# GothiProCoder/OCR-System

Hardware: AMD Instinct MI355X
Metric: pages/sec end-to-end det+rec, A4@200DPI (higher is better)
Workload: dtype bf16; 1 GPU; end-to-end det+rec, batch=64 A4@200DPI pages per GPU (BASELINE configs[3]); pages_per_gpu=64, global_batch=64, lines_last_step=3279, pages_gathered_last_step=64, parallelism=pages sharded dp1, 1 all-gather/step, ranks=1, input=pages pre-decoded (uint8 RGB) and resident in HBM when the timed region starts, det_sub_batch=64

## Files before the change

### ocr-system_amd/csrc/capi.hip

```cpp
#include <cstdlib>
#include <cstring>
#include <new>

#include "../../include/lumina_ocr.h"
#include "dbpost.h"
#include "deskew.h"
#include "engine.h"
#include "ops.h"
#include "resize.h"
#include "jpeg.h"
#include "jpegdec.h"
#include "stem_conv.h"

#define API_TRY try {
#define API_CATCH(h)                                                             \
    }                                                                            \
    catch (const std::exception& e) { return locr_fail(h, "exception", e.what()); } \
    catch (...) { return locr_fail(h, "exception", "unknown"); }

namespace {
struct DeviceGuard {
    int prev = -1;
    hipError_t err;
    explicit DeviceGuard(int dev) {
// ... 13 lines not shown

static int hip_rc(lumina_ocr* h, const char* what, hipError_t e) { return e == hipSuccess ? 0 : locr_fail(h, what, hipGetErrorString(e)); }

template <class F> static int drain_launches(lumina_ocr* h, const char* what, F&& f) {
    if (hipDeviceSynchronize() != hipSuccess) return locr_fail(h, what, "sync failed");
    for (const LaunchRecord& r : h->launches) {
        float t = 0.f;
        if (hipEventElapsedTime(&t, r.e0.get(), r.e1.get()) != hipSuccess) t = 0.f;
        f(r, t);
    }
    h->launches.clear();
    return 0;
}

extern "C" {

const char* lumina_ocr_version(void) { return "lumina-ocr-mi355x 0.1 (gfx950)"; }

int lumina_ocr_create(int device, lumina_ocr_t** out) {
    if (!out) return 1;
    *out = nullptr;
    lumina_ocr* eng = new (std::nothrow) lumina_ocr();
    if (!eng) return 1;
    eng->device = device;
    int ndev = 0;
    if (hipGetDeviceCount(&ndev) != hipSuccess || device < 0 || device >= ndev) {
        eng->err = "no HIP device " + std::to_string(device) + " (device count " + std::to_string(ndev) + ")";
        *out = eng;
        return 2;
    }
    if (hipSetDevice(device) != hipSuccess) { eng->err = "hipSetDevice failed"; *out = eng; return 2; }
    if (const char* e = getenv("LUMINA_RING_ORIENT")) eng->ring_orient = atoi(e) < 0 ? -1 : (atoi(e) != 0);
    if (getenv("LUMINA_CONV_NO_RING")) eng->conv_ring = false;
    if (getenv("LUMINA_BLOCKED")) eng->blocked_layout = atoi(getenv("LUMINA_BLOCKED")) != 0;
    *out = eng;
    return 0;
}

void lumina_ocr_destroy(lumina_ocr_t* h) {
    if (!h) return;
    (void)hipSetDevice(h->device);
    delete h;
}

const char* lumina_ocr_last_error(const lumina_ocr_t* h) { return h ? h->err.c_str() : "null handle"; }

int lumina_ocr_set_option(lumina_ocr_t* h, const char* key, int value) {
    if (!h || !key) return 1;
    if (!strcmp(key, "det_sub_batch")) h->det_sub_batch = value > 0 ? value : 1;
    else if (!strcmp(key, "rec_sub_batch")) h->rec_sub_batch = value > 0 ? value : 1;
    else if (!strcmp(key, "keep_taps")) h->keep_taps = value < 0 || value > 2 ? 0 : value;
    else if (!strcmp(key, "time_convs")) h->time_convs = value != 0;
    else if (!strcmp(key, "fuse_head")) h->fuse_head = value != 0;
    else if (!strcmp(key, "fuse_mb")) h->fuse_mb = value != 0;
    else if (!strcmp(key, "fuse_pool")) h->fuse_pool = value != 0;
    else if (!strcmp(key, "fuse_stem")) h->fuse_stem = value != 0;
    else if (!strcmp(key, "fpn_multi")) h->fpn_multi = value != 0;
    else if (!strcmp(key, "fpn_compose")) h->fpn_compose = value != 0;
    else if (!strcmp(key, "fuse_short")) h->fuse_short = value != 0;
    else if (!strcmp(key, "conv_ring")) h->conv_ring = value != 0;
    else if (!strcmp(key, "blocked_layout")) h->blocked_layout = value != 0;
    else if (!strcmp(key, "conv_big_min")) h->conv_big_min = value >= 0 ? value : 1024;
    else if (!strcmp(key, "ring_orient")) h->ring_orient = value < 0 ? -1 : (value != 0);
    else if (!strcmp(key, "post_group")) h->post_group = value > 0 ? value : 1;
    else if (!strcmp(key, "tail_group")) h->tail_group = value > 0 ? value : 0;
    else if (!strcmp(key, "svtr_f16")) h->svtr_f16 = value < 0 ? -1 : (value != 0);
    else if (!strcmp(key, "conv2d_variant")) h->conv2d_variant = value < 0 || value > 2 ? 0 : value;
    else return locr_fail(h, "set_option: unknown key", key);
    return 0;
}

int lumina_ocr_load_det_weights(lumina_ocr_t* h, const void* blob, size_t nbytes) {
    if (!h || !blob) return 1;
    BIND(h);
    API_TRY return eng_load_det(h, blob, nbytes); API_CATCH(h)
}
int lumina_ocr_load_rec_weights(lumina_ocr_t* h, const void* blob, size_t nbytes) {
    if (!h || !blob) return 1;
    BIND(h);
    API_TRY return eng_load_rec(h, blob, nbytes); API_CATCH(h)
}
int lumina_ocr_num_classes(const lumina_ocr_t* h) { return h ? h->num_classes : 0; }

int lumina_ocr_normalize(lumina_ocr_t* h, const uint8_t* img_dev, int n, int height, int width, int hp, int wp, const float scale[3],
                         const float shift[3], int layout_nchw, uint16_t* out_dev, void* stream) {
    if (!h || !img_dev || !out_dev || hp < height || wp < width) return locr_fail(h, "normalize", "bad arguments");
    BIND(h);
    return hip_rc(h, "normalize", normalize_launch(img_dev, out_dev, n, height, width, hp, wp, height, width, scale, shift, layout_nchw, (hipStream_t)stream));
}

int lumina_ocr_det_forward(lumina_ocr_t* h, const uint8_t* pages_dev, int batch, int height, int width, int hp, int wp, uint16_t* prob_dev,
                           void* stream) {
    if (!h || !pages_dev || !prob_dev) return locr_fail(h, "det_forward", "null argument");
// ... 327 lines not shown
```

### ocr-system_amd/csrc/conv_mfma.h

```cpp
#pragma once
#include "common.h"

enum ConvOutMode : int {
    OUT_NORMAL = 0,
    OUT_UPSAMPLE = 1,
    OUT_CONVT = 2,
    OUT_CONVT1 = 3,
    OUT_POOL = 4,
};

struct ConvParams {
    const bf16_t* x;
    const bf16_t* wpk;
    const float* bias;
    const bf16_t* res;
    bf16_t* y;
    int N, H, W, Cin;
    int Ho, Wo;
    int Cout;
    int y_cstride, y_coff;
    int res_cstride, res_h, res_w, res_shift;
    int act;
    int out_mode, up_shift, convt_c;
    int tiles_x, tiles_y, n_tiles;
// ... 1 lines not shown
    float fuse_b;
    const bf16_t* gate;
    int gate_hw;
    int dbg_skip;
    int pix_limit;
    const bf16_t* zeros;
    int x_blk, y_blk, res_blk;
    int n_src;
    const bf16_t* xs[4];
    int xs_shift[4];
    int xs_nchunk[4], xs_cstride[4];
    const bf16_t* wpk2;
    const float* bias2;
    bf16_t* y2;
    int y2_cstride;
};

struct ConvKernelCfg {
    int ks, stride, bn, ck, tw, nw;
};

size_t conv_packed_weight_elems(int cout_gemm, int ks, int cin, int bn);
void pack_conv_weights(const bf16_t* ohwi, int cout_gemm, int ks, int cin, int bn, int ck, bf16_t* out, int row_major = 0);

bool conv_pick_cfg(int ks, int stride, int cin, int cout_gemm, ConvKernelCfg* cfg);
hipError_t conv_launch(const ConvKernelCfg& cfg, ConvParams p, hipStream_t stream);
const char* conv_kernel_name(const ConvKernelCfg& cfg);

bool conv_ring_supported(const ConvKernelCfg& cfg, const ConvParams& p);
bool conv_ring_transposed(const ConvParams& p, int orientation);
hipError_t conv_ring_launch(ConvParams p, int orientation, hipStream_t stream);
const char* conv_ring_kernel_name(const ConvParams& p, int orientation);

bool conv_pw_supported(const ConvKernelCfg& cfg, const ConvParams& p);
hipError_t conv_pw_launch(const ConvParams& p, hipStream_t stream);
```

### ocr-system_amd/csrc/engine.h

```cpp
#pragma once
#include <map>
#include <memory>
#include <string>
#include <type_traits>
#include <vector>

#include "common.h"
#include "conv_mfma.h"
#include "mbconv.h"
#include "svtr.h"

struct Tensor4 {
    bf16_t* p = nullptr;
    int n = 0, h = 0, w = 0, c = 0;
    bool blk = false;
    int n_src = 0; const bf16_t* xs[4] = {nullptr, nullptr, nullptr, nullptr}; int xs_shift[4] = {0, 0, 0, 0};
    int xs_c[4] = {0, 0, 0, 0}, xs_cs[4] = {0, 0, 0, 0};
    int src_c(int k) const { return xs_c[k] ? xs_c[k] : c / n_src; }
    int src_cs(int k) const { return xs_cs[k] ? xs_cs[k] : src_c(k); }
    size_t elems() const { return (size_t)n * h * w * c; }
};

struct ConvLayer {
    std::string name;
    int ks = 1, stride = 1, cin = 0, cout = 0;
    int act = ACT_NONE;
    bool convt = false;
    int convt_c = 0;
    ConvKernelCfg cfg{};
    bf16_t* wpk = nullptr;
    ConvKernelCfg cfg_big{}; bf16_t* wpk_big = nullptr;
    bool force_big = false;
    int launch_group = 0;
    bool small_only = false;
    bf16_t* fuse_w = nullptr; float fuse_b = 0.f;
    double alg_flop_per_px = 0;
    float* bias = nullptr;
};

struct DwLayer { int k = 3, c = 0; bf16_t* w = nullptr; float* bias = nullptr; };
struct SeLayer { int c = 0, mid = 0; bf16_t *w1 = nullptr, *w2 = nullptr; float *b1 = nullptr, *b2 = nullptr; };

struct RecBlock {
    int k, cin, exp, cout, se_mid, stride_h, act;
    bool se, res;
    ConvLayer expand, project;
    DwLayer dw;
    bf16_t* we_pk = nullptr; float* be_pk = nullptr;
    SeLayer sel;
};

struct SvtrLinear {
    int K = 0, N = 0, taps = 1, cin = 0, act = ACT_NONE;
    uint16_t* w = nullptr;
    float* bias = nullptr;
    float *gamma = nullptr, *beta = nullptr;
};
struct SvtrBlock { int dim = 0, heads = 0, gh = 0, gw = 0; bool local = false; SvtrLinear qkv, proj, fc1, fc2; };
struct SvtrModel {
    bool loaded = false;
    int dtype = 0;
    int dims[3] = {64, 128, 256}, depths[3] = {3, 6, 3}, heads[3] = {2, 4, 8}, local_blocks = 6, out_ch = 192;
    int num_classes = 0, ctc_ntiles = 0;
    SvtrLinear pe1, pe2, sub[2], last;
// ... 31 lines not shown
struct HostBlobTensor { int dtype; std::vector<int> dims; const uint8_t* data; size_t nbytes; };

struct lumina_ocr {
    int device = 0;
    std::string err;
    bool det_loaded = false;
    std::map<std::string, ConvLayer> det;
    bf16_t* stem_wpk = nullptr; float* stem_bias = nullptr;
    bool rec_loaded = false;
    int num_classes = 0, ctc_ntiles = 0;
    bf16_t* rstem_wpk = nullptr; float* rstem_bias = nullptr;
    std::vector<RecBlock> rblocks;
    ConvLayer rconv2, xproj[2];
    bf16_t* whh[2] = {nullptr, nullptr};
    bf16_t* ctc_wpk = nullptr; float* ctc_bias = nullptr;
    SvtrModel svtr;
    Growable<DeviceMem> ws;
    Arena arena;
    std::vector<DeviceMem> owned;
    bf16_t* zeros = nullptr;
    int det_sub_batch = 16, rec_sub_batch = 4096, post_group = 64;
    int tail_group = 16;
    std::map<std::string, Tensor4> taps;
    int keep_taps = 0;
    bool fuse_head = true;
    bool fuse_pool = true;
    int conv_big_min = 1024;
    bool blocked_layout = true;
    bool conv_ring = true;
    int svtr_f16 = -1;
    int conv2d_variant = 0;
    int ring_orient = -1;
    bool fuse_short = true;
    bool fpn_compose = true;
    bool fpn_multi = true;
    bool fuse_stem = true;
    bool fuse_mb = true;
    bool time_convs = false;
    std::vector<LaunchRecord> launches;
    struct Coeffs { int ksize = 0; int* bounds = nullptr; int* kk = nullptr; std::shared_ptr<std::vector<int>> bounds_host; };
    std::map<std::pair<int, int>, Coeffs> coeff_cache;
    Growable<DeviceMem> aux;
    Growable<DeviceMem> sums;
    int jd_last_passes = 0;
    struct Staging { Growable<PinnedMem> buf; Event uploaded; };
    Staging jd_stage[2];
    int jd_stage_next = 0;
    float* dk_trig = nullptr; short* dk_wtab = nullptr;
};

int locr_fail(lumina_ocr* eng, const char* what, const char* detail);
bool parse_blob(lumina_ocr* eng, const void* blob, size_t n, std::map<std::string, HostBlobTensor>* out);

int eng_load_det(lumina_ocr* eng, const void* blob, size_t n);
int eng_load_rec(lumina_ocr* eng, const void* blob, size_t n);
int eng_det_forward(lumina_ocr* eng, const uint8_t* pages, int B, int H, int W, int Hp, int Wp, bf16_t* prob, hipStream_t st);
int eng_rec_forward(lumina_ocr* eng, const uint8_t* crops, const int* widths, int N, int* idx, float* prob, hipStream_t st);
int eng_load_svtr(lumina_ocr* eng, const void* blob, size_t n);
int eng_svtr_forward(lumina_ocr* eng, const uint8_t* crops, const int* widths, int N, int* idx, float* prob, hipStream_t st);
int eng_ws_reserve(lumina_ocr* eng, size_t bytes);
void* eng_upload(lumina_ocr* eng, const void* host, size_t bytes);
int eng_run_conv(lumina_ocr* eng, const ConvLayer& L, const Tensor4& x, Tensor4* y, const Tensor4* res, int res_shift, int out_mode,
                 int up_shift, int y_cstride, int y_coff, bool flat, hipStream_t st, const bf16_t* gate = nullptr,
                 const ConvLayer* short_l = nullptr, Tensor4* short_y = nullptr);
```

### ocr-system_amd/csrc/engine.hip

```cpp
#include "engine.h"

#include <cstdlib>
#include <cstring>

#include "ops.h"
#include "stem_conv.h"

int locr_fail(lumina_ocr* eng, const char* what, const char* detail) {
    if (eng) eng->err = std::string(what) + ": " + (detail ? detail : "");
    return 1;
}

#include <mutex>
#include <set>
hipError_t locr_dyn_lds(const void* kernel, int bytes) {
    static std::mutex mu;
    static std::set<std::pair<int, const void*>> done;
    int dev = 0;
    hipError_t e = hipGetDevice(&dev);
    if (e != hipSuccess) return e;
    std::lock_guard<std::mutex> lk(mu);
    if (done.count({dev, kernel})) return hipSuccess;
    e = hipFuncSetAttribute(kernel, hipFuncAttributeMaxDynamicSharedMemorySize, bytes);
    if (e == hipSuccess) done.insert({dev, kernel});
// ... 72 lines not shown
        locr_fail(eng, "missing/ill-typed tensor", name.c_str());
        return false;
    }
    *w = &iw->second; *b = &ib->second;
    return true;
}

static bool make_conv(lumina_ocr* eng, const std::map<std::string, HostBlobTensor>& m, const std::string& name, int ks, int stride,
                      int cin_r, int cout_r, int cin_p, int cout_p, int act, ConvLayer* L, int bias_repeat = 1) {
    const HostBlobTensor *w, *b;
    if (!get_wb(eng, m, name, &w, &b)) return false;
    if (w->dims.size() != 4 || w->dims[0] != cout_r || w->dims[1] != ks || w->dims[3] != cin_r ||
        (int)b->dims[0] * bias_repeat != cout_r) {
        locr_fail(eng, "unexpected tensor shape", name.c_str());
        return false;
    }
    L->name = name; L->ks = ks; L->stride = stride; L->cin = cin_p; L->cout = cout_p; L->act = act;
    if (!conv_pick_cfg(ks, stride, cin_p, cout_p, &L->cfg)) { locr_fail(eng, "no conv kernel config", name.c_str()); return false; }
    const int taps = ks * ks;
    std::vector<bf16_t> padded((size_t)cout_p * taps * cin_p, 0);
    const bf16_t* src = reinterpret_cast<const bf16_t*>(w->data);
    for (int co = 0; co < cout_r; ++co)
        for (int t = 0; t < taps; ++t)
            memcpy(&padded[((size_t)co * taps + t) * cin_p], &src[((size_t)co * taps + t) * cin_r], sizeof(bf16_t) * cin_r);
    std::vector<bf16_t> packed(conv_packed_weight_elems(cout_p, ks, cin_p, L->cfg.bn));
    pack_conv_weights(padded.data(), cout_p, ks, cin_p, L->cfg.bn, L->cfg.ck, packed.data());
    L->wpk = static_cast<bf16_t*>(eng_upload(eng, packed.data(), packed.size() * sizeof(bf16_t)));
    static const int dma = getenv("LUMINA_CONV_DMA") != nullptr ? atoi(getenv("LUMINA_CONV_DMA")) : 1;
    if (ks == 3 && stride == 1 && L->cfg.bn == 64 && (cin_p >= 64 || name == "stem.conv3") && L->cfg.nw == 4) {
        L->cfg_big = L->cfg; L->cfg_big.nw = dma ? 6 : 5; L->cfg_big.ck = 16;
        std::vector<bf16_t> packed2(conv_packed_weight_elems(cout_p, ks, cin_p, 64));
        pack_conv_weights(padded.data(), cout_p, ks, cin_p, 64, 16, packed2.data(), dma ? 1 : 0);
        L->wpk_big = static_cast<bf16_t*>(eng_upload(eng, packed2.data(), packed2.size() * sizeof(bf16_t)));
    }
    const int ntiles = (cout_p + L->cfg.bn - 1) / L->cfg.bn;
    std::vector<float> bias((size_t)ntiles * L->cfg.bn, 0.f);
    const float* bs = reinterpret_cast<const float*>(b->data);
    const int bn_r = b->dims[0];
    for (int i = 0; i < cout_r; ++i) bias[i] = bs[i % bn_r];
    L->bias = static_cast<float*>(eng_upload(eng, bias.data(), bias.size() * sizeof(float)));
    if (!L->wpk || !L->bias) { locr_fail(eng, "device upload failed", name.c_str()); return false; }
    return true;
}

static inline float host_bf16_to_f32(bf16_t b) { uint32_t u = (uint32_t)b << 16; float f; memcpy(&f, &u, 4); return f; }
static inline bf16_t host_f32_to_bf16(float f) {
    uint32_t u; memcpy(&u, &f, 4);
    return (bf16_t)((u + 0x7fffu + ((u >> 16) & 1u)) >> 16);
}

static int compose_fpn_p2(lumina_ocr* eng, const std::map<std::string, HostBlobTensor>& m) {
    const HostBlobTensor *wi, *bi, *wp, *bp;
    if (!get_wb(eng, m, "fpn.in2", &wi, &bi) || !get_wb(eng, m, "fpn.p2", &wp, &bp)) return 1;
    const float* b_in2 = reinterpret_cast<const float*>(bi->data);
    for (int i = 0; i < 256; ++i)
        if (b_in2[i] != 0.f) return 0;
    const bf16_t* Wi = reinterpret_cast<const bf16_t*>(wi->data);
    const bf16_t* Wp = reinterpret_cast<const bf16_t*>(wp->data);
    std::vector<bf16_t> w((size_t)64 * 9 * 320);
    std::vector<double> win((size_t)256 * 64);
    for (size_t i = 0; i < win.size(); ++i) win[i] = (double)host_bf16_to_f32(Wi[i]);
    for (int co = 0; co < 64; ++co)
        for (int t = 0; t < 9; ++t) {
            double acc[64] = {0};
            const bf16_t* row = Wp + ((size_t)co * 9 + t) * 256;
            for (int mm = 0; mm < 256; ++mm) {
// ... 59 lines not shown
        ConvLayer& L3 = eng->det["head.convt3"];
        if (!make_conv(eng, m, "head.convt3", 1, 1, 64, 4, 64, 4, ACT_SIGMOID, &L3, 4)) return 1;
        L3.convt = true; L3.convt_c = 1;
        const HostBlobTensor *w3, *b3;
        if (!get_wb(eng, m, "head.convt3", &w3, &b3)) return 1;
        ConvLayer& Lf = eng->det["head.convt2.fused"];
        Lf = L;
        Lf.name = "head.convt2+3";
        {
            const bf16_t* w3s = reinterpret_cast<const bf16_t*>(w3->data);
            std::vector<bf16_t> img(4 * 2 * 32 * 8, 0);
            for (int ks = 0; ks < 4; ++ks)
                for (int hh = 0; hh < 2; ++hh)
                    for (int row = 0; row < 4; ++row)
                        for (int j = 0; j < 8; ++j) img[((ks * 2 + hh) * 32 + row) * 8 + j] = w3s[row * 64 + ks * 16 + hh * 8 + j];
            Lf.fuse_w = static_cast<bf16_t*>(eng_upload(eng, img.data(), img.size() * sizeof(bf16_t)));
        }
        Lf.fuse_b = reinterpret_cast<const float*>(b3->data)[0];
        if (!Lf.fuse_w) return locr_fail(eng, "upload", "head.convt3 fused weights");
    }
    eng->det_loaded = true;
    return 0;
}

static bool conv_takes_big(const lumina_ocr* eng, const ConvLayer& L, int n, int ho, int wo, bool flat) {
    static const bool no_big = getenv("LUMINA_CONV_NO_BIG") != nullptr;
    static const long long big_min_env = getenv("LUMINA_CONV_BIG_MIN") ? atoll(getenv("LUMINA_CONV_BIG_MIN")) : -1;
    const long long nb_eff = n > eng->det_sub_batch ? n : eng->det_sub_batch;
    const long long big_blocks = nb_eff * ((ho + 15) / 16) * ((wo + 31) / 32) * ((L.cout + L.cfg.bn - 1) / L.cfg.bn);
    const long long big_min = big_min_env >= 0 ? big_min_env : eng->conv_big_min;
    return (L.force_big && L.wpk_big != nullptr) || (!no_big && !flat && !L.small_only && L.wpk_big != nullptr && big_blocks >= big_min);
}

struct LaunchTimer {
    lumina_ocr* eng; hipStream_t st; Event e0, e1;
    LaunchTimer(lumina_ocr* e, hipStream_t s, bool enabled = true) : eng(e), st(s) {
        if (!enabled || !e->time_convs) return;
        hipEvent_t a = nullptr, b = nullptr;
        if (hipEventCreate(&a) == hipSuccess) e0.reset(a);
        if (hipEventCreate(&b) == hipSuccess) e1.reset(b);
        if (!e0 || !e1 || hipEventRecord(e0.get(), st) != hipSuccess) { e0.reset(); e1.reset(); }
    }
    bool on() const { return e1 != nullptr; }
    void done(std::string layer, std::string kernel, double flop, double bytes) {
        if (!on() || hipEventRecord(e1.get(), st) != hipSuccess) return;
        eng->launches.push_back(LaunchRecord{std::move(e0), std::move(e1), flop, bytes, std::move(layer), std::move(kernel)});
    }
};

int eng_run_conv(lumina_ocr* eng, const ConvLayer& L, const Tensor4& x, Tensor4* y, const Tensor4* res, int res_shift, int out_mode,
                 int up_shift, int y_cstride, int y_coff, bool flat, hipStream_t st, const bf16_t* gate, const ConvLayer* short_l, Tensor4* short_y) {
    if (short_l != nullptr && L.launch_group > 0) return locr_fail(eng, "fused shortcut", "not available with launch groups");
    if (L.launch_group > 0 && x.n > L.launch_group && !flat && gate == nullptr && x.p != nullptr && y->p != nullptr &&
        (out_mode == OUT_NORMAL) && !x.blk && !y->blk && (!res || !res->blk)) {
        ConvLayer one = L;
        one.launch_group = 0;
        const size_t ystride = (size_t)y->h * y->w * (y_cstride ? y_cstride : y->c);
        for (int b0 = 0; b0 < x.n; b0 += L.launch_group) {
            const int nb = x.n - b0 < L.launch_group ? x.n - b0 : L.launch_group;
            Tensor4 xs = x, ys = *y, rs;
            xs.n = nb; xs.p = x.p + (size_t)b0 * x.h * x.w * (x.n_src > 1 ? x.src_cs(x.n_src - 1) : x.c);
            for (int k = 0; k < x.n_src; ++k) xs.xs[k] = x.xs[k] + (size_t)b0 * (x.h >> x.xs_shift[k]) * (x.w >> x.xs_shift[k]) * x.src_cs(k);
            ys.n = nb; ys.p = y->p + (size_t)b0 * ystride;
            if (res) { rs = *res; rs.n = nb; rs.p = res->p + (size_t)b0 * res->h * res->w * res->c; }
            if (eng_run_conv(eng, one, xs, &ys, res ? &rs : nullptr, res_shift, out_mode, up_shift, y_cstride, y_coff, flat, st, gate)) return 1;
        }
// ... 7 lines not shown
    p.Cin = L.cin; p.Cout = L.cout; p.act = L.act;
    p.out_mode = out_mode; p.up_shift = up_shift; p.convt_c = L.convt_c;
    p.fuse_w = (out_mode == OUT_CONVT) ? L.fuse_w : nullptr; p.fuse_b = L.fuse_b;
    if (flat) {
        const long long m = (long long)x.n * x.h * x.w;
        p.N = 1; p.W = 32; p.H = (int)((m + 31) / 32); p.pix_limit = (int)m;
        p.Ho = p.H; p.Wo = 32;
        p.res_h = p.H; p.res_w = 32;
    } else {
        p.N = x.n; p.H = x.h; p.W = x.w; p.pix_limit = 0;
        p.Ho = (L.ks == 3) ? (x.h - 1) / L.stride + 1 : x.h / L.stride;
        p.Wo = (L.ks == 3) ? (x.w - 1) / L.stride + 1 : x.w / L.stride;
        if (res) { p.res_h = res->h; p.res_w = res->w; }
    }
    p.res_shift = res_shift;
    p.x_blk = x.blk; p.y_blk = y->blk; p.res_blk = res ? res->blk : 0;
    p.n_src = x.n_src;
    for (int k = 0; k < 4; ++k) {
        p.xs[k] = x.xs[k]; p.xs_shift[k] = x.xs_shift[k];
        p.xs_nchunk[k] = k < x.n_src ? x.src_c(k) / 16 : 0; p.xs_cstride[k] = k < x.n_src ? x.src_cs(k) : 0;
    }
    p.res_cstride = res ? res->c : 0;
    p.y_cstride = y_cstride ? y_cstride : y->c;
    p.y_coff = y_coff;
    if (short_l != nullptr) {
        if (short_y == nullptr || short_l->cin != L.cin || short_l->cout != L.cout || short_l->cfg.bn != L.cfg.bn || short_l->cfg.ck != L.cfg.ck ||
            short_l->ks != 2 || short_l->stride != 2 || short_y->c != L.cout || short_y->h != y->h || short_y->w != y->w)
            return locr_fail(eng, "fused shortcut: layer mismatch", L.name.c_str());
        p.wpk2 = short_l->wpk; p.bias2 = short_l->bias; p.y2 = short_y->p; p.y2_cstride = short_y->c;
    }
    if (x.c != L.cin) return locr_fail(eng, "conv input channels mismatch", L.name.c_str());
    if (x.p == nullptr || y->p == nullptr) return ws_null(eng, L.name.c_str());
    LaunchTimer tm(eng, st);
    if (out_mode == OUT_POOL && (L.wpk_big == nullptr || L.cfg_big.nw != 6)) return locr_fail(eng, "fused max pool needs the LDS-DMA conv kernel", L.name.c_str());
    const bool use_big = out_mode == OUT_POOL || p.n_src > 1 || conv_takes_big(eng, L, p.N, p.Ho, p.Wo, flat);
    if (L.force_big && eng->conv2d_variant == 2 && !conv_ring_supported(L.cfg_big, p)) return locr_fail(eng, "conv2d_variant 2: the ring kernel does not take this layer", L.name.c_str());
    ConvKernelCfg cfg = L.cfg;
    if (use_big) { cfg = L.cfg_big; p.wpk = L.wpk_big; }
    static const bool no_pw = getenv("LUMINA_CONV_NO_PW") != nullptr;
    const bool use_pw = !no_pw && !use_big && conv_pw_supported(cfg, p);
    const bool use_ring = eng->conv_ring && use_big && !use_pw && conv_ring_supported(cfg, p);
    if (p.n_src > 1 && !use_ring) return locr_fail(eng, "a multi-source input reached a kernel other than the ring kernel", L.name.c_str());
    if (!use_ring && (p.x_blk || p.y_blk || p.res_blk)) return locr_fail(eng, "a channel-blocked tensor reached a kernel that cannot address it", L.name.c_str());
    hipError_t e = use_ring ? conv_ring_launch(p, eng->ring_orient, st) : (use_pw ? conv_pw_launch(p, st) : conv_launch(cfg, p, st));
    if (e != hipSuccess) return locr_fail(eng, L.name.c_str(), hipGetErrorString(e));
    if (tm.on()) {
        const double px = flat ? (double)p.pix_limit : (double)p.N * p.Ho * p.Wo;
        const double flop = (L.alg_flop_per_px > 0 ? px * L.alg_flop_per_px : 2.0 * px * L.ks * L.ks * L.cin * L.cout) +
                            (short_l ? 2.0 * px * 4 * short_l->cin * short_l->cout : 0.0);
        double in_elems = (double)x.elems();
        if (x.n_src > 1) { in_elems = 0; for (int k = 0; k < x.n_src; ++k) in_elems += (double)x.n * (x.h >> x.xs_shift[k]) * (x.w >> x.xs_shift[k]) * x.src_c(k); }
        const double bytes = 2.0 * (in_elems + px * (out_mode == OUT_CONVT && p.fuse_w ? 4.0 : (double)L.cout) * (out_mode == OUT_UPSAMPLE ? (double)(1 << (2 * up_shift)) : (out_mode == OUT_POOL ? 0.25 : 1.0)) + (res ? px * (double)L.cout / (double)(1 << (2 * res_shift)) : 0.0) + (double)L.ks * L.ks * L.cin * L.cout +
                                    (short_l ? px * (double)short_l->cout + 4.0 * short_l->cin * short_l->cout : 0.0));
        std::string kname = use_pw ? (L.cin == 64 ? "conv_pw_kernel<64>" : "conv_pw_kernel<128>") : conv_kernel_name(cfg);
        if (use_ring) kname = conv_ring_kernel_name(p, eng->ring_orient);
        if (short_l) { const size_t pos = kname.rfind(",0,2>"); if (pos != std::string::npos) kname.replace(pos, 5, ",5,2>"); }
        if (out_mode == OUT_POOL && !use_ring) { const size_t pos = kname.rfind(",3,4>"); if (pos != std::string::npos) kname.replace(pos, 5, ",4,4>"); }
        tm.done(short_l ? L.name + "+short" : L.name, kname, flop, bytes);
    }
    return 0;
}

#define RUN(expr) do { if ((expr) != 0) return 1; } while (0)

static void tap(lumina_ocr* eng, const char* name, const Tensor4& t) { if (eng->keep_taps && t.p) eng->taps[name] = t; }

// ... 24 lines not shown
    if (!fuse_pool || dry) t3 = ws_tensor(eng, B, Hp / 2, Wp / 2, 64);
    Tensor4 x = ws_tensor(eng, B, Hp / 4, Wp / 4, 64);
    if (fuse_pool) {
        RUN(eng_run_conv(eng, D["stem.conv3"], t2, &x, nullptr, 0, OUT_POOL, 0, 0, 0, false, st));
    } else {
        RUN(eng_run_conv(eng, D["stem.conv3"], t2, &t3, nullptr, 0, OUT_NORMAL, 0, 0, 0, false, st)); tap(eng, "stem.conv3", t3);
        if (!dry && x.p) {
            hipError_t e = maxpool_launch(t3.p, x.p, B, t3.h, t3.w, 64, 3, 2, 1, x.h, x.w, st);
            if (e != hipSuccess) return locr_fail(eng, "stem.pool", hipGetErrorString(e));
        }
    }
    tap(eng, "stem.pool", x);
    const int chs[4] = {64, 128, 256, 512};
    Tensor4 feats[4];
    for (int i = 0; i < 4; ++i) {
        for (int j = 0; j < 2; ++j) {
            const std::string p = "s" + std::to_string(i) + ".b" + std::to_string(j);
            const int stride = (i > 0 && j == 0) ? 2 : 1;
            Tensor4 y = ws_tensor(eng, B, x.h / stride, x.w / stride, chs[i]);
            const bool blk = i == 0 && eng->blocked_layout && eng->keep_taps == 0 && eng->conv_ring && !dry &&
                             conv_takes_big(eng, D[p + ".conv0"], B, x.h, x.w, false) && conv_takes_big(eng, D[p + ".conv1"], B, x.h, x.w, false);
            y.blk = blk;
            const ConvLayer& c0 = D[p + ".conv0"];
            const bool fuse_sc = eng->fuse_short && i > 0 && j == 0 && x.h % 2 == 0 && x.w % 2 == 0 && c0.cfg.bn == 64 && c0.cfg.ck == 16 && c0.cfg.nw == 4 &&
                                 D[p + ".short"].cfg.bn == 64 && D[p + ".short"].cfg.ck == 16;
            Tensor4 sc = x;
            if (j == 0) sc = ws_tensor(eng, B, y.h, y.w, chs[i]);
            if (fuse_sc) {
                RUN(eng_run_conv(eng, c0, x, &y, nullptr, 0, OUT_NORMAL, 0, 0, 0, false, st, nullptr, &D[p + ".short"], &sc));
            } else {
                RUN(eng_run_conv(eng, c0, x, &y, nullptr, 0, OUT_NORMAL, 0, 0, 0, false, st));
                if (j == 0) RUN(eng_run_conv(eng, D[p + ".short"], x, &sc, nullptr, 0, OUT_NORMAL, 0, 0, 0, i == 0, st));
            }
            Tensor4 o = ws_tensor(eng, B, y.h, y.w, chs[i]);
            o.blk = blk && j == 0;
            RUN(eng_run_conv(eng, D[p + ".conv1"], y, &o, &sc, 0, OUT_NORMAL, 0, 0, 0, false, st));
            tap(eng, p.c_str(), o);
            x = o;
        }
        feats[i] = x;
    }
    Tensor4 in5 = ws_tensor(eng, B, feats[3].h, feats[3].w, 256);
    RUN(eng_run_conv(eng, D["fpn.in5"], feats[3], &in5, nullptr, 0, OUT_NORMAL, 0, 0, 0, false, st));
    Tensor4 out4 = ws_tensor(eng, B, feats[2].h, feats[2].w, 256);
    RUN(eng_run_conv(eng, D["fpn.in4"], feats[2], &out4, &in5, 1, OUT_NORMAL, 0, 0, 0, false, st));
    Tensor4 out3 = ws_tensor(eng, B, feats[1].h, feats[1].w, 256);
    RUN(eng_run_conv(eng, D["fpn.in3"], feats[1], &out3, &out4, 1, OUT_NORMAL, 0, 0, 0, false, st));
    ConvLayer& hc1 = D["head.conv1"];
    const bool multi = eng->fpn_multi && eng->keep_taps != 1 && eng->conv_ring && conv_takes_big(eng, hc1, B, Hp / 4, Wp / 4, false) &&
                       (Hp / 4) % 8 == 0 && (Wp / 4) % 8 == 0;
    auto slice = [](const Tensor4& t, int b0, int nb) {
        Tensor4 r = t;
        r.n = nb;
        if (t.p) r.p = t.p + (size_t)b0 * t.h * t.w * t.c;
        return r;
    };
    const bool compose = eng->fpn_compose && eng->conv_ring && D.count("fpn.p2c") != 0;
    auto run_p2 = [&](const Tensor4& c2, const Tensor4& o3, Tensor4* lateral, Tensor4* dst, int y_cstride, int y_coff) -> int {
        if (compose) {
            Tensor4 in = c2;
            in.c = 320; in.n_src = 2;
            in.xs[0] = c2.p; in.xs[1] = o3.p; in.p = o3.p;
            in.xs_shift[0] = 0; in.xs_shift[1] = 1; in.xs_c[0] = 64; in.xs_c[1] = 256;
            return eng_run_conv(eng, D["fpn.p2c"], in, dst, nullptr, 0, OUT_NORMAL, 0, y_cstride, y_coff, false, st);
        }
        RUN(eng_run_conv(eng, D["fpn.in2"], c2, lateral, &o3, 1, OUT_NORMAL, 0, 0, 0, false, st));
// ... 501 lines not shown
```

Baseline: 1527 pages/sec.

## Add fused stride-2 ring conv kernel computing stage-entry conv0 and shortcut together

Adds a new persistent LDS-DMA MFMA kernel for stride-2 3x3 convolutions that also computes the 2x2 stride-2 shortcut conv from the same staged input halo, writing both outputs. It is used for backbone stage-entry blocks with enough channels and tiles, so the input is read once for both convolutions and one launch is dropped. The kernel double-buffers input and weight chunks and interleaves DMA issue with the MFMA schedule. It adds extra packed weight copies and a large new kernel whose tile shape and occupancy may not beat the existing fused-shortcut path on all layer sizes.

```diff
diff --git a/ocr-system_amd/csrc/capi.hip b/ocr-system_amd/csrc/capi.hip
--- a/ocr-system_amd/csrc/capi.hip
+++ b/ocr-system_amd/csrc/capi.hip
@@ -69,6 +69,7 @@
     if (hipSetDevice(device) != hipSuccess) { eng->err = "hipSetDevice failed"; *out = eng; return 2; }
     if (const char* e = getenv("LUMINA_RING_ORIENT")) eng->ring_orient = atoi(e) < 0 ? -1 : (atoi(e) != 0);
     if (getenv("LUMINA_CONV_NO_RING")) eng->conv_ring = false;
+    if (getenv("LUMINA_CONV_NO_RING_S2")) eng->ring_s2 = false;
     if (getenv("LUMINA_BLOCKED")) eng->blocked_layout = atoi(getenv("LUMINA_BLOCKED")) != 0;
     *out = eng;
     return 0;
@@ -96,6 +97,9 @@
     else if (!strcmp(key, "fpn_compose")) h->fpn_compose = value != 0;
     else if (!strcmp(key, "fuse_short")) h->fuse_short = value != 0;
     else if (!strcmp(key, "conv_ring")) h->conv_ring = value != 0;
+    else if (!strcmp(key, "ring_s2")) h->ring_s2 = value != 0;
+    else if (!strcmp(key, "ring_s2_min")) h->ring_s2_min = value >= 0 ? value : 1536;
+    else if (!strcmp(key, "ring_s2_cin")) h->ring_s2_cin = value >= 0 ? value : 128;
     else if (!strcmp(key, "blocked_layout")) h->blocked_layout = value != 0;
     else if (!strcmp(key, "conv_big_min")) h->conv_big_min = value >= 0 ? value : 1024;
     else if (!strcmp(key, "ring_orient")) h->ring_orient = value < 0 ? -1 : (value != 0);
diff --git a/ocr-system_amd/csrc/conv_mfma.h b/ocr-system_amd/csrc/conv_mfma.h
--- a/ocr-system_amd/csrc/conv_mfma.h
+++ b/ocr-system_amd/csrc/conv_mfma.h
@@ -57,5 +57,10 @@
 hipError_t conv_ring_launch(ConvParams p, int orientation, hipStream_t stream);
 const char* conv_ring_kernel_name(const ConvParams& p, int orientation);
 
+bool conv_ring_s2_supported(const ConvParams& p);
+bool conv_ring_s2_transposed(const ConvParams& p, int orientation);
+hipError_t conv_ring_s2_launch(ConvParams p, int orientation, hipStream_t stream);
+const char* conv_ring_s2_kernel_name(const ConvParams& p, int orientation);
+
 bool conv_pw_supported(const ConvKernelCfg& cfg, const ConvParams& p);
 hipError_t conv_pw_launch(const ConvParams& p, hipStream_t stream);
diff --git a/ocr-system_amd/csrc/conv_ring_s2.hip b/ocr-system_amd/csrc/conv_ring_s2.hip
--- /dev/null
+++ b/ocr-system_amd/csrc/conv_ring_s2.hip
@@ -0,0 +1,308 @@
+#include "conv_mfma.h"
+
+#include <cstdlib>
+
+namespace {
+
+constexpr int S2_TH = 8, S2_TW = 32, S2_HH = 2 * S2_TH + 1, S2_HW = 2 * S2_TW + 1, S2_BN = 64, S2_MT = 2, S2_NT = 2, S2_NTHR = 256;
+constexpr int S2_A_ITEMS = S2_HH * S2_HW * 2;
+constexpr int S2_AIT = (S2_A_ITEMS + S2_NTHR - 1) / S2_NTHR;
+constexpr int S2_A_BYTES = S2_AIT * S2_NTHR * 16;
+constexpr int S2_W_ITEMS = 9 * S2_BN * 2, S2_WIT = (S2_W_ITEMS + S2_NTHR - 1) / S2_NTHR;
+constexpr int S2_W2_ITEMS = 4 * S2_BN * 2, S2_W2IT = S2_W2_ITEMS / S2_NTHR;
+constexpr int S2_W_BYTES = S2_W_ITEMS * 16, S2_W2_BYTES = S2_W2_ITEMS * 16;
+constexpr int S2_BUF = S2_A_BYTES + S2_W_BYTES + S2_W2_BYTES;
+constexpr int S2_COUT_MAX = 512;
+constexpr int S2_LDS = 2 * S2_BUF + 2 * S2_COUT_MAX * 4;
+constexpr int S2_NDMA = S2_AIT + S2_WIT + S2_W2IT;
+static_assert(S2_LDS <= 160 * 1024 && S2_W2_ITEMS % S2_NTHR == 0 && S2_W_ITEMS % 64 == 0, "LDS budget / whole-wave requests");
+
+__device__ __forceinline__ int s2_slot(int pi, int c) { return 2 * (pi ^ ((pi >> 3) & 1)) + (c ^ ((pi >> 4) & 1)); }
+__device__ __forceinline__ bf16x8_t s2_frag(const unsigned char* p) { return *reinterpret_cast<const bf16x8_t*>(p); }
+
+struct S2Tile { int n_img, ntile, oyb, oxb; };
+
+template <int TR>
+__global__ __launch_bounds__(S2_NTHR, 1) void conv_ring_s2_kernel(const ConvParams p, const int total_tiles, const int per_xcd, const int wg_per_xcd) {
+    extern __shared__ __attribute__((aligned(16))) unsigned char smem[];
+    const int tid = threadIdx.x, lane = tid & 63, wave = __builtin_amdgcn_readfirstlane(tid >> 6), r = lane & 31, h = lane >> 5;
+
+    const int LH = TR ? p.W : p.H, LW = TR ? p.H : p.W, LHo = TR ? p.Wo : p.Ho, LWo = TR ? p.Ho : p.Wo;
+    const int sy = TR ? 1 : p.W, sx = TR ? p.W : 1, osy = TR ? 1 : p.Wo, osx = TR ? p.Wo : 1;
+    const int tiles_per_img = p.tiles_x * p.tiles_y;
+    const int nchunks = p.Cin >> 4;
+
+    const int xcd = blockIdx.x & 7;
+    int lid = xcd * per_xcd + (blockIdx.x >> 3);
+    const int lid_end = min((xcd + 1) * per_xcd, total_tiles);
+    if (lid >= lid_end) return;
+
+    auto decode = [&](int id) {
+        S2Tile t;
+        t.ntile = id % p.n_tiles;
+        const int mtile = id / p.n_tiles;
+        t.n_img = mtile / tiles_per_img;
+        const int trem = mtile - t.n_img * tiles_per_img;
+        const int ty = trem / p.tiles_x;
+        t.oyb = ty * S2_TH; t.oxb = (trem - ty * p.tiles_x) * S2_TW;
+        return t;
+    };
+
+    unsigned a_item[(S2_AIT + 1) / 2];
+#pragma unroll
+    for (int it = 0; it < S2_AIT; ++it) {
+        const int i = tid + S2_NTHR * it, pi = (i >> 1) ^ ((i >> 4) & 1), c = (i & 1) ^ ((i >> 5) & 1);
+        const int hy = pi / S2_HW, hx = pi - hy * S2_HW;
+        const unsigned e = (unsigned)hy | ((unsigned)hx << 5) | ((unsigned)c << 12) | ((unsigned)(pi < S2_HH * S2_HW) << 13);
+        if (it & 1) a_item[it >> 1] |= e << 16; else a_item[it >> 1] = e;
+    }
+    int a_goff[S2_AIT];
+    auto describe = [&](const S2Tile& t) {
+#pragma unroll
+        for (int j = 0; j < (S2_AIT + 1) / 2; ++j) asm volatile("" : "+v"(a_item[j]));
+#pragma unroll
+        for (int it = 0; it < S2_AIT; ++it) {
+            const unsigned e = (a_item[it >> 1] >> (16 * (it & 1))) & 0xffffu;
+            const int hy = e & 31, hx = (e >> 5) & 127, c = (e >> 12) & 1;
+            const int ly = 2 * t.oyb - 1 + hy, lx = 2 * t.oxb - 1 + hx;
+            const bool inb = (e >> 13) != 0 && ly >= 0 && ly < LH && lx >= 0 && lx < LW;
+            a_goff[it] = inb ? (ly * sy + lx * sx) * p.Cin + c * 8 : -1;
+        }
+    };
+    const bf16_t *ximg, *wbase, *wbase2;
+    auto rebase = [&](const S2Tile& t) {
+        ximg = p.x + (size_t)t.n_img * p.H * p.W * p.Cin;
+        wbase = p.wpk + (size_t)t.ntile * nchunks * (S2_W_ITEMS * 8);
+        wbase2 = p.wpk2 + (size_t)t.ntile * nchunks * (S2_W2_ITEMS * 8);
+    };
+
+    auto dma_a = [&](int it, const bf16_t* xa, int tgt) {
+        const unsigned long long in_addr = (unsigned long long)xa + 2ull * (unsigned)a_goff[it];
+        const unsigned long long addr = a_goff[it] >= 0 ? in_addr : (unsigned long long)p.zeros;
+        __builtin_amdgcn_global_load_lds((const __attribute__((address_space(1))) void*)addr,
+            (__attribute__((address_space(3))) void*)(smem + tgt + (wave * 64 + S2_NTHR * it) * 16), 16, 0, 0);
+    };
+    auto dma_w = [&](int it, const bf16_t* wsrc, int tgt) {
+        const int i = tid + S2_NTHR * it;
+        if (S2_W_ITEMS % S2_NTHR == 0 || (it + 1) * S2_NTHR <= S2_W_ITEMS || wave < (S2_W_ITEMS % S2_NTHR) / 64)
+            __builtin_amdgcn_global_load_lds((const __attribute__((address_space(1))) void*)(wsrc + (i ^ ((i >> 4) & 1)) * 8),
+                (__attribute__((address_space(3))) void*)(smem + S2_A_BYTES + tgt + (wave * 64 + S2_NTHR * it) * 16), 16, 0, 0);
+    };
+    auto dma_w2 = [&](int it, const bf16_t* wsrc, int tgt) {
+        const int i = tid + S2_NTHR * it;
+        __builtin_amdgcn_global_load_lds((const __attribute__((address_space(1))) void*)(wsrc + (i ^ ((i >> 4) & 1)) * 8),
+            (__attribute__((address_space(3))) void*)(smem + S2_A_BYTES + S2_W_BYTES + tgt + (wave * 64 + S2_NTHR * it) * 16), 16, 0, 0);
+    };
+    auto dma_k = [&](int k, const bf16_t* xa, const bf16_t* ws, const bf16_t* ws2, int tgt) {
+        if (k < S2_AIT) dma_a(k, xa, tgt);
+        else if (k < S2_AIT + S2_WIT) dma_w(k - S2_AIT, ws, tgt);
+        else dma_w2(k - S2_AIT - S2_WIT, ws2, tgt);
+    };
+
+    f32x16_t acc[S2_MT][S2_NT], acc2[S2_MT][S2_NT];
+    const f32x16_t zero16 = {0.f, 0.f, 0.f, 0.f, 0.f, 0.f, 0.f, 0.f, 0.f, 0.f, 0.f, 0.f, 0.f, 0.f, 0.f, 0.f};
+    int aoff[S2_MT][9];
+#pragma unroll
+    for (int mt = 0; mt < S2_MT; ++mt)
+#pragma unroll
+        for (int lt = 0; lt < 9; ++lt) {
+            const int pi = (2 * (wave * S2_MT + mt) + lt / 3) * S2_HW + 2 * r + lt % 3;
+            aoff[mt][lt] = 16 * s2_slot(pi, h);
+        }
+    const int woff = S2_A_BYTES + r * 32 + 16 * (h ^ ((r >> 3) & 1));
+    const int woff2 = woff + S2_W_BYTES;
+
+    bf16x8_t bfr[2][S2_MT], afr[2][S2_NT], a2[2][S2_NT];
+#define S2_LT(tap_) (TR ? ((tap_) % 3) * 3 + (tap_) / 3 : (tap_))
+#define S2_SC(tap_) ((tap_) == 4 || (tap_) == 5 || (tap_) == 7 || (tap_) == 8)
+#define S2_T2(tap_) ((tap_) == 4 ? 0 : (tap_) == 5 ? 1 : (tap_) == 7 ? 2 : 3)
+#define S2_FRAGS(boff_, tap_, set_)                                                                                \
+    {                                                                                                              \
+        _Pragma("unroll") for (int mt = 0; mt < S2_MT; ++mt) bfr[set_][mt] = s2_frag(smem + (boff_) + aoff[mt][S2_LT(tap_)]); \
+        _Pragma("unroll") for (int nt = 0; nt < S2_NT; ++nt) afr[set_][nt] = s2_frag(smem + (boff_) + woff + ((tap_) * S2_BN + nt * 32) * 32); \
+    }
+#define S2_COMPUTE(boff_, tgt_, first_)                                                                            \
+    S2_FRAGS(boff_, 0, 0)                                                                                          \
+    __builtin_amdgcn_sched_barrier(0);                                                                             \
+    _Pragma("unroll") for (int st = 0; st < 9; ++st) {                                                             \
+        const int nx_ = (st + 1) & 1, tapn_ = st + 1;                                                              \
+        const int nf_ = S2_SC(st) ? 8 : 4;                                                                         \
+        int m0_ = 0;                                                                                               \
+        _Pragma("unroll") for (int u = 0; u < st; ++u) m0_ += S2_SC(u) ? 8 : 4;    \
+        _Pragma("unroll") for (int q_ = 0; q_ < nf_; ++q_) {                                                       \
+            if (q_ < 4) {                                                                                          \
+                const int mt = q_ / S2_NT, nt = q_ % S2_NT;                                                        \
+                acc[mt][nt] = __builtin_amdgcn_mfma_f32_32x32x16_bf16(afr[st & 1][nt], bfr[st & 1][mt], ((first_) && st == 0) ? zero16 : acc[mt][nt], 0, 0, 0); \
+            } else {                                                                                               \
+                const int mt = (q_ - 4) / S2_NT, nt = (q_ - 4) % S2_NT;                                            \
+                acc2[mt][nt] = __builtin_amdgcn_mfma_f32_32x32x16_bf16(a2[st & 1][nt], bfr[st & 1][mt], ((first_) && st == 4) ? zero16 : acc2[mt][nt], 0, 0, 0); \
+            }                                                                                                      \
+            __builtin_amdgcn_sched_barrier(0);                                                                     \
+            if (st + 1 < 9) {                                                                                      \
+                if (q_ == 0) { _Pragma("unroll") for (int nt = 0; nt < S2_NT; ++nt) afr[nx_][nt] = s2_frag(smem + (boff_) + woff + (tapn_ * S2_BN + nt * 32) * 32); } \
+                if (q_ == 1) { _Pragma("unroll") for (int mt = 0; mt < S2_MT; ++mt) bfr[nx_][mt] = s2_frag(smem + (boff_) + aoff[mt][S2_LT(tapn_)]); } \
+                if (q_ == 2 && S2_SC(tapn_)) { _Pragma("unroll") for (int nt = 0; nt < S2_NT; ++nt) a2[nx_][nt] = s2_frag(smem + (boff_) + woff2 + (S2_T2(tapn_) * S2_BN + nt * 32) * 32); } \
+            }                                                                                                      \
+            if (st < 7) {                                                                                          \
+                _Pragma("unroll") for (int k = 0; k < S2_NDMA; ++k)                                                \
+                    if (k * 36 / S2_NDMA == m0_ + q_) dma_k(k, xa_n, ws_n, ws2_n, tgt_);                           \
+            }                                                                                                      \
+            __builtin_amdgcn_sched_barrier(0);                                                                     \
+        }                                                                                                          \
+    }
+
+    uint4 pk[S2_MT][S2_NT][2], pk2[S2_MT][S2_NT][2];
+    S2Tile done{};
+    bool pending = false;
+    auto store_done = [&]() {
+        const size_t img = (size_t)done.n_img * p.Ho * p.Wo;
+        const int co = done.ntile * S2_BN + 8 * h;
+        const int ox = done.oxb + r;
+#pragma unroll
+        for (int mt = 0; mt < S2_MT; ++mt) {
+            const int oy = done.oyb + wave * S2_MT + mt;
+            if (oy >= LHo || ox >= LWo) continue;
+            const size_t pix = img + oy * osy + ox * osx;
+            bf16_t* ypix = p.y + pix * p.y_cstride + p.y_coff + co;
+            bf16_t* y2pix = p.y2 + pix * p.y2_cstride + co;
+#pragma unroll
+            for (int nt = 0; nt < S2_NT; ++nt)
+#pragma unroll
+                for (int gp = 0; gp < 2; ++gp) {
+                    *reinterpret_cast<uint4*>(ypix + nt * 32 + 16 * gp) = pk[mt][nt][gp];
+                    *reinterpret_cast<uint4*>(y2pix + nt * 32 + 16 * gp) = pk2[mt][nt][gp];
+                }
+        }
+    };
+
+    float* sBias = reinterpret_cast<float*>(smem + 2 * S2_BUF);
+    float* sBias2 = sBias + S2_COUT_MAX;
+    S2Tile cur{};
+    auto epilogue = [&]() {
+        int hb = h;
+        asm volatile("" : "+v"(hb));
+        const float* bsrc = sBias + cur.ntile * S2_BN + 4 * hb;
+        const float* bsrc2 = sBias2 + cur.ntile * S2_BN + 4 * hb;
+#pragma unroll
+        for (int mt = 0; mt < S2_MT; ++mt) {
+            __builtin_amdgcn_sched_barrier(0);
+#pragma unroll
+            for (int nt = 0; nt < S2_NT; ++nt)
+#pragma unroll
+                for (int g = 0; g < 4; ++g) {
+                    const float4 b4 = *reinterpret_cast<const float4*>(bsrc + nt * 32 + 8 * g);
+                    float v0 = acc[mt][nt][4 * g + 0] + b4.x, v1 = acc[mt][nt][4 * g + 1] + b4.y;
+                    float v2 = acc[mt][nt][4 * g + 2] + b4.z, v3 = acc[mt][nt][4 * g + 3] + b4.w;
+                    if (p.act == ACT_RELU) { v0 = fmaxf(v0, 0.f); v1 = fmaxf(v1, 0.f); v2 = fmaxf(v2, 0.f); v3 = fmaxf(v3, 0.f); }
+                    acc[mt][nt][4 * g + 0] = v0; acc[mt][nt][4 * g + 1] = v1; acc[mt][nt][4 * g + 2] = v2; acc[mt][nt][4 * g + 3] = v3;
+                    const float4 c4 = *reinterpret_cast<const float4*>(bsrc2 + nt * 32 + 8 * g);
+                    acc2[mt][nt][4 * g + 0] += c4.x; acc2[mt][nt][4 * g + 1] += c4.y; acc2[mt][nt][4 * g + 2] += c4.z; acc2[mt][nt][4 * g + 3] += c4.w;
+                }
+#pragma unroll
+            for (int nt = 0; nt < S2_NT; ++nt)
+#pragma unroll
+                for (int gp = 0; gp < 2; ++gp) {
+                    const int g0 = 2 * gp, g1 = 2 * gp + 1;
+                    {
+                        const uint32_t q0x = pack_bf16x2(acc[mt][nt][4 * g0 + 0], acc[mt][nt][4 * g0 + 1]), q0y = pack_bf16x2(acc[mt][nt][4 * g0 + 2], acc[mt][nt][4 * g0 + 3]);
+                        const uint32_t q1x = pack_bf16x2(acc[mt][nt][4 * g1 + 0], acc[mt][nt][4 * g1 + 1]), q1y = pack_bf16x2(acc[mt][nt][4 * g1 + 2], acc[mt][nt][4 * g1 + 3]);
+                        const auto sx2 = __builtin_amdgcn_permlane32_swap(q0x, q1x, false, false);
+                        const auto sy2 = __builtin_amdgcn_permlane32_swap(q0y, q1y, false, false);
+                        pk[mt][nt][gp] = make_uint4(sx2[0], sy2[0], sx2[1], sy2[1]);
+                    }
+                    {
+                        const uint32_t q0x = pack_bf16x2(acc2[mt][nt][4 * g0 + 0], acc2[mt][nt][4 * g0 + 1]), q0y = pack_bf16x2(acc2[mt][nt][4 * g0 + 2], acc2[mt][nt][4 * g0 + 3]);
+                        const uint32_t q1x = pack_bf16x2(acc2[mt][nt][4 * g1 + 0], acc2[mt][nt][4 * g1 + 1]), q1y = pack_bf16x2(acc2[mt][nt][4 * g1 + 2], acc2[mt][nt][4 * g1 + 3]);
+                        const auto sx2 = __builtin_amdgcn_permlane32_swap(q0x, q1x, false, false);
+                        const auto sy2 = __builtin_amdgcn_permlane32_swap(q0y, q1y, false, false);
+                        pk2[mt][nt][gp] = make_uint4(sx2[0], sy2[0], sx2[1], sy2[1]);
+                    }
+                }
+            __builtin_amdgcn_sched_barrier(0);
+        }
+    };
+
+    for (int i = tid; i < p.Cout; i += S2_NTHR) { sBias[i] = p.bias[i]; sBias2[i] = p.bias2[i]; }
+    cur = decode(lid);
+    S2Tile nxt = cur;
+    describe(cur); rebase(cur);
+    int boff = 0;
+    const bf16_t* xa_n = ximg;
+    const bf16_t* ws_n = wbase;
+    const bf16_t* ws2_n = wbase2;
+#pragma unroll
+    for (int k = 0; k < S2_NDMA; ++k) dma_k(k, xa_n, ws_n, ws2_n, 0);
+    for (;;) {
+        const int next_lid = lid + wg_per_xcd;
+        asm volatile("s_waitcnt vmcnt(0)" ::: "memory");
+        __syncthreads();
+        xa_n += 16; ws_n += S2_W_ITEMS * 8; ws2_n += S2_W2_ITEMS * 8;
+        if (pending) store_done();
+        S2_COMPUTE(boff, S2_BUF - boff, true)
+        boff = S2_BUF - boff;
+        for (int chunk = 1; chunk < nchunks; ++chunk) {
+            asm volatile("s_waitcnt vmcnt(0)" ::: "memory");
+            __syncthreads();
+            if (chunk + 1 < nchunks) {
+                xa_n += 16; ws_n += S2_W_ITEMS * 8; ws2_n += S2_W2_ITEMS * 8;
+            } else if (next_lid < lid_end) {
+                nxt = decode(next_lid);
+                describe(nxt); rebase(nxt);
+                xa_n = ximg; ws_n = wbase; ws2_n = wbase2;
+            }
+            S2_COMPUTE(boff, S2_BUF - boff, false)
+            boff = S2_BUF - boff;
+        }
+        epilogue();
+        done = cur; pending = true;
+        lid = next_lid;
+        if (lid >= lid_end) break;
+        cur = nxt;
+    }
+    asm volatile("s_waitcnt vmcnt(0)" ::: "memory");
+    store_done();
+#undef S2_COMPUTE
+#undef S2_FRAGS
+#undef S2_T2
+#undef S2_SC
+#undef S2_LT
+}
+
+}
+
+bool conv_ring_s2_supported(const ConvParams& p) {
+    static const bool off = getenv("LUMINA_CONV_NO_RING_S2") != nullptr;
+    if (off) return false;
+    if (p.wpk == nullptr || p.wpk2 == nullptr || p.bias2 == nullptr || p.y2 == nullptr || p.zeros == nullptr) return false;
+    if (p.out_mode != OUT_NORMAL || p.pix_limit != 0 || p.gate != nullptr || p.res != nullptr || p.n_src > 1 || p.x_blk || p.y_blk) return false;
+    if (p.act != ACT_NONE && p.act != ACT_RELU) return false;
+    if (p.Cin < 32 || p.Cin % 16 != 0 || p.Cout % S2_BN != 0 || p.Cout > S2_COUT_MAX) return false;
+    if (p.H % 2 != 0 || p.W % 2 != 0 || p.Ho != p.H / 2 || p.Wo != p.W / 2) return false;
+    if (p.y_cstride % 8 != 0 || p.y_coff % 8 != 0 || p.y2_cstride % 8 != 0 || p.y_coff + p.Cout > p.y_cstride || p.Cout > p.y2_cstride) return false;
+    if ((long long)p.H * p.W * p.Cin >= (1ll << 31)) return false;
+    return true;
+}
+
+bool conv_ring_s2_transposed(const ConvParams& p, int orientation) {
+    auto padded = [&](int lh, int lw) { return (long long)ceil_div(lh, S2_TH) * S2_TH * ceil_div(lw, S2_TW) * S2_TW; };
+    return orientation < 0 ? padded(p.Wo, p.Ho) < padded(p.Ho, p.Wo) : orientation != 0;
+}
+
+const char* conv_ring_s2_kernel_name(const ConvParams& p, int orientation) {
+    return conv_ring_s2_transposed(p, orientation) ? "conv_ring_s2_kernel<1>" : "conv_ring_s2_kernel<0>";
+}
+
+hipError_t conv_ring_s2_launch(ConvParams p, int orientation, hipStream_t stream) {
+    if (!conv_ring_s2_supported(p)) return hipErrorInvalidValue;
+    const bool tr = conv_ring_s2_transposed(p, orientation);
+    p.tiles_y = ceil_div(tr ? p.Wo : p.Ho, S2_TH); p.tiles_x = ceil_div(tr ? p.Ho : p.Wo, S2_TW); p.n_tiles = p.Cout / S2_BN;
+    const long long total = (long long)p.N * p.tiles_x * p.tiles_y * p.n_tiles;
+    if (total <= 0 || total >= (1ll << 31)) return hipErrorInvalidValue;
+    const int per_xcd = (int)((total + 7) / 8);
+    const int wg_per_xcd = per_xcd < 32 ? per_xcd : 32;
+    const void* fn = tr ? reinterpret_cast<const void*>(conv_ring_s2_kernel<1>) : reinterpret_cast<const void*>(conv_ring_s2_kernel<0>);
+    { hipError_t e = locr_dyn_lds(fn, S2_LDS); if (e != hipSuccess) return e; }
+    if (tr) hipLaunchKernelGGL((conv_ring_s2_kernel<1>), dim3(8 * wg_per_xcd), dim3(S2_NTHR), S2_LDS, stream, p, (int)total, per_xcd, wg_per_xcd);
+    else hipLaunchKernelGGL((conv_ring_s2_kernel<0>), dim3(8 * wg_per_xcd), dim3(S2_NTHR), S2_LDS, stream, p, (int)total, per_xcd, wg_per_xcd);
+    return hipGetLastError();
+}
diff --git a/ocr-system_amd/csrc/engine.h b/ocr-system_amd/csrc/engine.h
--- a/ocr-system_amd/csrc/engine.h
+++ b/ocr-system_amd/csrc/engine.h
@@ -30,6 +30,7 @@
     ConvKernelCfg cfg{};
     bf16_t* wpk = nullptr;
     ConvKernelCfg cfg_big{}; bf16_t* wpk_big = nullptr;
+    bf16_t* wpk_s2 = nullptr;
     bool force_big = false;
     int launch_group = 0;
     bool small_only = false;
@@ -127,6 +128,9 @@
     int conv2d_variant = 0;
     int ring_orient = -1;
     bool fuse_short = true;
+    bool ring_s2 = true;
+    int ring_s2_min = 1536;
+    int ring_s2_cin = 128;
     bool fpn_compose = true;
     bool fpn_multi = true;
     bool fuse_stem = true;
diff --git a/ocr-system_amd/csrc/engine.hip b/ocr-system_amd/csrc/engine.hip
--- a/ocr-system_amd/csrc/engine.hip
+++ b/ocr-system_amd/csrc/engine.hip
@@ -128,6 +128,12 @@
         std::vector<bf16_t> packed2(conv_packed_weight_elems(cout_p, ks, cin_p, 64));
         pack_conv_weights(padded.data(), cout_p, ks, cin_p, 64, 16, packed2.data(), dma ? 1 : 0);
         L->wpk_big = static_cast<bf16_t*>(eng_upload(eng, packed2.data(), packed2.size() * sizeof(bf16_t)));
+    }
+    if (stride == 2 && (ks == 3 || ks == 2) && L->cfg.bn == 64 && L->cfg.ck == 16) {
+        std::vector<bf16_t> packed2(conv_packed_weight_elems(cout_p, ks, cin_p, 64));
+        pack_conv_weights(padded.data(), cout_p, ks, cin_p, 64, 16, packed2.data(), 1);
+        L->wpk_s2 = static_cast<bf16_t*>(eng_upload(eng, packed2.data(), packed2.size() * sizeof(bf16_t)));
+        if (!L->wpk_s2) { locr_fail(eng, "device upload failed", name.c_str()); return false; }
     }
     const int ntiles = (cout_p + L->cfg.bn - 1) / L->cfg.bn;
     std::vector<float> bias((size_t)ntiles * L->cfg.bn, 0.f);
@@ -253,6 +259,12 @@
     return (L.force_big && L.wpk_big != nullptr) || (!no_big && !flat && !L.small_only && L.wpk_big != nullptr && big_blocks >= big_min);
 }
 
+static bool entry_takes_ring(const lumina_ocr* eng, const ConvLayer& L, const ConvLayer& S, int n, int ho, int wo) {
+    if (!eng->ring_s2 || L.wpk_s2 == nullptr || S.wpk_s2 == nullptr || L.cin < eng->ring_s2_cin) return false;
+    const long long nb_eff = n > eng->det_sub_batch ? n : eng->det_sub_batch;
+    return nb_eff * ((ho + 7) / 8) * ((wo + 31) / 32) * ((L.cout + 63) / 64) >= eng->ring_s2_min;
+}
+
 struct LaunchTimer {
     lumina_ocr* eng; hipStream_t st; Event e0, e1;
     LaunchTimer(lumina_ocr* e, hipStream_t s, bool enabled = true) : eng(e), st(s) {
@@ -326,6 +338,21 @@
     if (x.c != L.cin) return locr_fail(eng, "conv input channels mismatch", L.name.c_str());
     if (x.p == nullptr || y->p == nullptr) return ws_null(eng, L.name.c_str());
     LaunchTimer tm(eng, st);
+    if (short_l != nullptr && entry_takes_ring(eng, L, *short_l, p.N, p.Ho, p.Wo)) {
+        ConvParams q = p;
+        q.wpk = L.wpk_s2; q.wpk2 = short_l->wpk_s2;
+        if (conv_ring_s2_supported(q)) {
+            hipError_t e = conv_ring_s2_launch(q, eng->ring_orient, st);
+            if (e != hipSuccess) return locr_fail(eng, L.name.c_str(), hipGetErrorString(e));
+            if (tm.on()) {
+                const double px = (double)p.N * p.Ho * p.Wo;
+                const double flop = 2.0 * px * (9.0 + 4.0) * L.cin * L.cout;
+                const double bytes = 2.0 * ((double)x.elems() + 2.0 * px * L.cout + 13.0 * L.cin * L.cout);
+                tm.done(L.name + "+short", conv_ring_s2_kernel_name(q, eng->ring_orient), flop, bytes);
+            }
+            return 0;
+        }
+    }
     if (out_mode == OUT_POOL && (L.wpk_big == nullptr || L.cfg_big.nw != 6)) return locr_fail(eng, "fused max pool needs the LDS-DMA conv kernel", L.name.c_str());
     const bool use_big = out_mode == OUT_POOL || p.n_src > 1 || conv_takes_big(eng, L, p.N, p.Ho, p.Wo, flat);
     if (L.force_big && eng->conv2d_variant == 2 && !conv_ring_supported(L.cfg_big, p)) return locr_fail(eng, "conv2d_variant 2: the ring kernel does not take this layer", L.name.c_str());
@@ -416,6 +443,7 @@
                 RUN(eng_run_conv(eng, c0, x, &y, nullptr, 0, OUT_NORMAL, 0, 0, 0, false, st));
                 if (j == 0) RUN(eng_run_conv(eng, D[p + ".short"], x, &sc, nullptr, 0, OUT_NORMAL, 0, 0, 0, i == 0, st));
             }
+            if (j == 0 && i > 0) { tap(eng, (p + ".conv0").c_str(), y); tap(eng, (p + ".short").c_str(), sc); }
             Tensor4 o = ws_tensor(eng, B, y.h, y.w, chs[i]);
             o.blk = blk && j == 0;
             RUN(eng_run_conv(eng, D[p + ".conv1"], y, &o, &sc, 0, OUT_NORMAL, 0, 0, 0, false, st));
```

After: 1537 pages/sec (median of 6 runs). About the same (+0.6%).
